# DuckTapeDevOps/kubernetes-cloud

Hardware: AMD Instinct MI355X
Metric: GPT-J-6B finetune tokens/sec (higher is better)
Workload: dtype bf16; 1 GPU; model=gpt-j-6b, global_batch=32, micro_batch=16, grad_accum=2, seq_len=2048, parallelism=dp1, activation_checkpointing=False

## Files before the change

csrc/kernels/attention_tiled.hip:

```cpp
#include "common.h"

#include <type_traits>

namespace {

constexpr float kLog2e = 1.4426950408889634f;
constexpr float kLn2 = 0.6931471805599453f;
constexpr float kRescaleThr = 8.0f;

#ifdef KCA_ATTN_STAMPS
__device__ unsigned long long g_attn_stamps[64];
__device__ __forceinline__ unsigned long long ast_now() {
  unsigned long long t;
  __builtin_amdgcn_sched_barrier(0);
  asm volatile("s_memtime %0\n\ts_waitcnt lgkmcnt(0)" : "=s"(t)::"memory");
  __builtin_amdgcn_sched_barrier(0);
  return t;
}
#define ASTAMP_DECL                                            \
  unsigned long long st_acc_[8] = {0, 0, 0, 0, 0, 0, 0, 0}; \
  unsigned long long st_prev_ = ast_now();
#define ASTAMP(k)                           \
  do {                                      \
    const unsigned long long n_ = ast_now(); \
    st_acc_[k] += n_ - st_prev_;            \
    st_prev_ = n_;                          \
  } while (0)
#define ASTAMP_FLUSH(base)                                                          \
  do {                                                                              \
    st_acc_[7] = 1;                                                                 \
    if ((threadIdx.x & 63) == 0)                                                    \
      for (int i_ = 0; i_ < 8; ++i_) atomicAdd(&g_attn_stamps[(base) + i_], st_acc_[i_]); \
  } while (0)
#else
#define ASTAMP_DECL
#define ASTAMP(k) \
  do {            \
  } while (0)
#define ASTAMP_FLUSH(base) \
  do {                     \
  } while (0)
#endif


struct FastFwdParams {
  const bf16_t* q; const bf16_t* k; const bf16_t* v;
  bf16_t* o; float* lse;
  int* flags;
  long long q_sb, q_st, q_sh, k_sb, k_st, k_sh, v_sb, v_st, v_sh;
  long long o_sb, o_st, o_sh;
  int B, Sq, Sk, H, Hkv;
  float scale;
};

typedef __attribute__((address_space(3))) bf16x4 lds_bf16x4_t;
typedef unsigned int u32x4 __attribute__((ext_vector_type(4)));

__device__ __forceinline__ bf16x4 lds_tr4(const char* base, int byte_off) {
  return __builtin_amdgcn_ds_read_tr16_b64_v4bf16(
      (lds_bf16x4_t*)(reinterpret_cast<uintptr_t>(base + byte_off)));
}

__device__ __forceinline__ bf16x8 lds_b128(const char* base, int byte_off) {
  return *reinterpret_cast<const bf16x8*>(base + byte_off);
}

template <int D>
__device__ __forceinline__ int img_off(int row, int ch) {
// ... 409 lines not shown
  u32x4 r;
#if defined(__HIP_DEVICE_COMPILE__)
  asm volatile("ds_read_b128 %0, %1 offset:%2" : "=v"(r) : "v"(addr), "i"(OFF));
#endif
  return r;
}
template <int OFF>
__device__ __forceinline__ u32x2 ads_tr(unsigned addr) {
  u32x2 r;
#if defined(__HIP_DEVICE_COMPILE__)
  asm volatile("ds_read_b64_tr_b16 %0, %1 offset:%2" : "=v"(r) : "v"(addr), "i"(OFF));
#endif
  return r;
}
template <int N>
__device__ __forceinline__ void lgkm_wait(u32x4& x) {
#if defined(__HIP_DEVICE_COMPILE__)
  asm volatile("s_waitcnt lgkmcnt(%1)" : "+v"(x) : "n"(N));
#endif
}
template <int N>
__device__ __forceinline__ void lgkm_wait(u32x2& x, u32x2& y, u32x2& z, u32x2& w) {
#if defined(__HIP_DEVICE_COMPILE__)
  asm volatile("s_waitcnt lgkmcnt(%4)" : "+v"(x), "+v"(y), "+v"(z), "+v"(w) : "n"(N));
#endif
}
__device__ __forceinline__ bf16x8 as_bf8(u32x4 x) { return *reinterpret_cast<bf16x8*>(&x); }
__device__ __forceinline__ bf16x8 as_bf8(u32x2 lo, u32x2 hi) {
  u32x4 x{lo[0], lo[1], hi[0], hi[1]};
  return *reinterpret_cast<bf16x8*>(&x);
}

template <int D, bool CAUSAL, int NW = 8, int NBUF = 4>
__global__ void __launch_bounds__(NW * 64, 1) attn_fwd_w8_kernel(FastFwdParams p) {
  constexpr int BM = NW * 32, BN = 32;
  constexpr int TILE = BN * D * 2;
  constexpr int STAGE = 2 * TILE;
  constexpr int KS = D / 16;
  constexpr int PIECES = TILE / 1024;
  constexpr int PPW = PIECES / NW;
  constexpr int LEAD = NBUF - 1;
  constexpr int INFLIGHT = (LEAD - 1) * 2 * PPW;
  static_assert(((D == 256 || D == 128) && NW == 8) || (D == 512 && NW == 4 && NBUF == 2 && !CAUSAL),
                "multi-wave LDS-DMA forward: 8 waves at D = 128 / 256, 4 waves at D = 512");
  static_assert(PPW >= 1 && PIECES % NW == 0, "whole pieces per wave");
  constexpr int SMEM = (NBUF * STAGE > NW * 32 * D * 2) ? NBUF * STAGE : NW * 32 * D * 2;
  __shared__ __attribute__((aligned(1024))) char smem[SMEM];

  const int tid = threadIdx.x, lane = tid & 63;
  const int wave = __builtin_amdgcn_readfirstlane(tid >> 6);
  const int l32 = lane & 31, hh = lane >> 5;
  const int nqb = p.Sq / BM;
  const int lid = xcd_remap(blockIdx.x, gridDim.x);
  const int qi = lid % nqb;
  const int qb = CAUSAL ? (nqb - 1 - qi) : qi;
  const int bh = lid / nqb;
  const int b = bh / p.H, h = bh % p.H;
  const int hk = h / (p.H / p.Hkv);
  const int off = p.Sk - p.Sq;
  const int q0 = qb * BM + wave * 32;
  const int qrow = q0 + l32;
  int kv_hi = p.Sk;
  if (CAUSAL) kv_hi = min(kv_hi, qb * BM + BM + off);
  const int ntiles = kv_hi / BN;
  const int mytiles = CAUSAL ? min(ntiles, (q0 + 32 + off) / BN) : ntiles;
  const float sl2 = p.scale * kLog2e;

  const bf16_t* qp = p.q + b * p.q_sb + h * p.q_sh;
  bf16x8 qf[KS];
#pragma unroll
  for (int s = 0; s < KS; ++s)
    qf[s] = *reinterpret_cast<const bf16x8*>(qp + (long long)qrow * p.q_st + 16 * s + 8 * hh);
  asm volatile("s_waitcnt vmcnt(0)" ::: "memory");

  const __amdgpu_buffer_rsrc_t rk = head_rsrc(p.k + b * p.k_sb + hk * p.k_sh);
  const __amdgpu_buffer_rsrc_t rv = head_rsrc(p.v + b * p.v_sb + hk * p.v_sh);
  static_assert((D / 64) % PPW == 0, "a wave's pieces within one row group");
  int kvo, vvo;
  {
    const int byte = 1024 * (wave * PPW) + 16 * lane;
    const int rg = byte / (16 * D), rem = byte % (16 * D);
    const int chh = rem / 512, w5 = rem % 512;
    const int row = rg * 8 + w5 / 64;
    const int ch = chh * 4 + (((w5 % 64) / 16) ^ ((row >> 2) & 3));
    kvo = (int)(((long long)row * p.k_st + ch * 8) * 2);
    vvo = (int)(((long long)row * p.v_st + ch * 8) * 2);
  }
  typedef __attribute__((address_space(3))) char lds_char;
  lds_char* lsm = (lds_char*)smem;
// ... 299 lines not shown
    {
      bf16x8 t0[2], t1[2];
      t0[0] = tr_frag<D>(Ks, b1, b2, 0, 0);
      t1[0] = tr_frag<D>(Ks, b1, b2, 1, 0);
      __builtin_amdgcn_sched_group_barrier(0x100, 4, 0);
#pragma unroll
      for (int db = 0; db < D / 32; ++db) {
        if (db + 1 < D / 32) {
          t0[(db + 1) & 1] = tr_frag<D>(Ks, b1, b2, 0, db + 1);
          t1[(db + 1) & 1] = tr_frag<D>(Ks, b1, b2, 1, db + 1);
          __builtin_amdgcn_sched_group_barrier(0x100, 4, 0);
        }
        dq[db] = __builtin_amdgcn_mfma_f32_32x32x16_bf16(t0[db & 1], d0, dq[db], 0, 0, 0);
        dq[db] = __builtin_amdgcn_mfma_f32_32x32x16_bf16(t1[db & 1], d1, dq[db], 0, 0, 0);
        __builtin_amdgcn_sched_group_barrier(0x8, 2, 0);
      }
    }
    ASTAMP(4);
    asm volatile("" ::: "memory");
    if (t + 1 < ntiles) stg.store(sk, sv, smem + ((t + 1) & 1) * 2 * TILE);
    __syncthreads();
    ASTAMP(5);
  };
  const int nfree = CAUSAL ? ntiles - 4 : ntiles;
  for (int t = 0; t < nfree; ++t) tile_step(t, std::false_type{});
  for (int t = max(nfree, 0); t < ntiles; ++t) tile_step(t, std::true_type{});
  store_tile_lds<D, DS>(p.dq + b * p.dq_sb + h * p.dq_sh + (long long)q0 * p.dq_st, p.dq_st, dq, lane, p.scale,
                        smem + wave * 32 * D * 2);
  ASTAMP(6);
  ASTAMP_FLUSH(16);
}

template <int D, bool CAUSAL>
__global__ void __launch_bounds__(256, 2) attn_bwd_dq_ds_kernel(FastBwdWsParams p) {
  constexpr int BM = 128, BN = 32;
  constexpr int TILE = BN * D * 2;
  constexpr int NCH = D / 8, CPT = 32 * NCH / 256, RPI = 256 / NCH;
  constexpr int DST = BN * 32 * 2;
  constexpr int DOFF = 2 * TILE;
  __shared__ __attribute__((aligned(16))) char smem[4 * TILE];
  static_assert(DOFF + 2 * 4 * DST <= 4 * TILE && 256 % NCH == 0, "dQ from dS: LDS plan");

  const int tid = threadIdx.x, lane = tid & 63, wave = tid >> 6;
  const int hh = lane >> 5;
  const int nqb = p.Sq / BM;
  const int lid = xcd_remap(blockIdx.x, gridDim.x);
  const int qi = lid % nqb;
  const int qb = CAUSAL ? (nqb - 1 - qi) : qi;
  const int bh = lid / nqb;
  const int b = bh / p.H, h = bh % p.H;
  const int off = p.Sk - p.Sq;
  const int q0 = qb * BM + wave * 32;
  int kv_hi = p.Sk;
  if (CAUSAL) kv_hi = min(kv_hi, qb * BM + BM + off);
  const int ntiles = (kv_hi + BN - 1) / BN;

  f32x16 dq[D / 32];
#pragma unroll
  for (int i = 0; i < D / 32; ++i)
#pragma unroll
    for (int r = 0; r < 16; ++r) dq[i][r] = 0.f;

  const __amdgpu_buffer_rsrc_t rk = head_rsrc(p.k + b * p.k_sb + h * p.k_sh);
  int vok[CPT], lk[CPT];
#pragma unroll
  for (int i = 0; i < CPT; ++i) {
    vok[i] = (int)(((long long)(tid / NCH + i * RPI) * p.k_st + (tid % NCH) * 8) * 2);
    lk[i] = img_off<D>(tid / NCH + i * RPI, tid % NCH);
  }
  const __amdgpu_buffer_rsrc_t rw = head_rsrc(p.ws + (long long)bh * p.Sq * p.Sk);
  const int ws_row = __builtin_amdgcn_readfirstlane((q0 / 32) * (p.Sk / 32) * DST);
  const int wv = lane * 16;
  char* const dsl = smem + DOFF + wave * DST;
  int dsw[4], dsr[4];
#pragma unroll
  for (int n = 0; n < 4; ++n) {
    const int l32 = lane & 31, key = 8 * n + 4 * hh + ((lane & 15) >> 2), qq = 4 * ((lane >> 4) & 1) + (lane & 3);
    dsw[n] = 64 * l32 + 8 * ((hh + 2 * n) ^ (l32 >> 2));
    dsr[n] = 64 * key + 8 * (qq ^ (key >> 2));
  }
  int b1, b2;
  tr_bases<D>(lane, b1, b2);

  constexpr int PD = 2;
  u32x4 sk[CPT], sd[PD][2];
  auto load_k = [&](int t) {
    const int sok = __builtin_amdgcn_readfirstlane((int)(t * BN * p.k_st * 2));
#pragma unroll
    for (int i = 0; i < CPT; ++i) {
      const auto a = __builtin_amdgcn_raw_buffer_load_b128(rk, vok[i], sok, 0);
      sk[i] = *reinterpret_cast<const u32x4*>(&a);
    }
  };
  auto load_ds = [&](int t, auto set) {
    const int so = __builtin_amdgcn_readfirstlane(ws_row + t * DST);
#pragma unroll
    for (int i = 0; i < 2; ++i) {
      const auto a = __builtin_amdgcn_raw_buffer_load_b128(rw, wv, so + i * (DST / 2), 2);
      sd[decltype(set)::value][i] = *reinterpret_cast<const u32x4*>(&a);
    }
  };
  auto store_tile = [&](int buf, auto set) {
    constexpr int J = decltype(set)::value;
#pragma unroll
    for (int i = 0; i < CPT; ++i) *reinterpret_cast<u32x4*>(smem + buf * TILE + lk[i]) = sk[i];
#pragma unroll
    for (int i = 0; i < 2; ++i) {
      *reinterpret_cast<u32x2*>(dsl + buf * 4 * DST + dsw[2 * i]) = u32x2{sd[J][i][0], sd[J][i][1]};
      *reinterpret_cast<u32x2*>(dsl + buf * 4 * DST + dsw[2 * i + 1]) = u32x2{sd[J][i][2], sd[J][i][3]};
    }
  };
  const int last = ntiles - 1;

  load_k(0);
  load_ds(0, std::integral_constant<int, 0>{});
  store_tile(0, std::integral_constant<int, 0>{});
  static_for<1, PD>([&](auto T) { load_ds(min(decltype(T)::value, last), T); });
  __builtin_amdgcn_sched_barrier(0);
  load_k(min(1, last));
  __builtin_amdgcn_sched_barrier(0);
  load_ds(min(PD, last), std::integral_constant<int, 0>{});
  __syncthreads();
  auto tile_step = [&](int t, auto jc) {
    constexpr int NX = (decltype(jc)::value + 1) % PD;
    const char* Ks = smem + (t & 1) * TILE;
    const char* ds = dsl + (t & 1) * 4 * DST;
    const bf16x8 d0 = cat8(lds_tr4(ds, dsr[0]), lds_tr4(ds, dsr[1]));
    const bf16x8 d1 = cat8(lds_tr4(ds, dsr[2]), lds_tr4(ds, dsr[3]));
    {
      bf16x8 t0[2], t1[2];
      t0[0] = tr_frag<D>(Ks, b1, b2, 0, 0);
      t1[0] = tr_frag<D>(Ks, b1, b2, 1, 0);
      __builtin_amdgcn_sched_group_barrier(0x100, 8, 0);
#pragma unroll
      for (int db = 0; db < D / 32; ++db) {
        if (db + 1 < D / 32) {
          t0[(db + 1) & 1] = tr_frag<D>(Ks, b1, b2, 0, db + 1);
          t1[(db + 1) & 1] = tr_frag<D>(Ks, b1, b2, 1, db + 1);
          __builtin_amdgcn_sched_group_barrier(0x100, 4, 0);
        }
        dq[db] = __builtin_amdgcn_mfma_f32_32x32x16_bf16(t0[db & 1], d0, dq[db], 0, 0, 0);
        dq[db] = __builtin_amdgcn_mfma_f32_32x32x16_bf16(t1[db & 1], d1, dq[db], 0, 0, 0);
        __builtin_amdgcn_sched_group_barrier(0x8, 2, 0);
      }
    }
    asm volatile("" ::: "memory");
    if (t + 1 < ntiles) store_tile((t + 1) & 1, std::integral_constant<int, NX>{});
    load_k(min(t + 2, last));
    load_ds(min(t + 1 + PD, last), std::integral_constant<int, NX>{});
    __syncthreads();
  };
  for (int t = 0; t < ntiles; t += PD)
    static_for<0, PD>([&](auto J) { tile_step(t + decltype(J)::value, J); });
  store_tile_lds<D>(p.dq + b * p.dq_sb + h * p.dq_sh + (long long)q0 * p.dq_st, p.dq_st, dq, lane, p.scale,
                    smem + wave * 32 * D * 2);
}

template <int D, bool CAUSAL, int DS = D>
__global__ void __launch_bounds__(256, (D <= 64 && !CAUSAL) ? 3 : 1) attn_bwd_dkdv_tiled_kernel(FastBwdParams p) {
  constexpr int BK = 128, BQ = 32;
  constexpr int TILE = BQ * D * 2;
  using Stg = StagerFor<D, DS>;
  constexpr int NCH = D / 8, NCS = DS / 8, CPT = Stg::CPT;
  constexpr int KSD = DS / 16;
  constexpr int VOFF = 4 * TILE;
  constexpr int LOFF = VOFF + 4 * TILE;
  __shared__ __attribute__((aligned(16))) char smem[LOFF + 2 * 64 * 4];
  ASTAMP_DECL

  const int tid = threadIdx.x, lane = tid & 63, wave = tid >> 6;
  const int l32 = lane & 31, hh = lane >> 5;
  const int nkb = p.Sk / BK;
  const int lid = xcd_remap(blockIdx.x, gridDim.x);
  const int kb = lid % nkb, bh = lid / nkb;
  const int b = bh / p.Hkv, hk = bh % p.Hkv;
  const int grp = p.H / p.Hkv;
  const int off = p.Sk - p.Sq;
  const int kw = kb * BK + wave * 32;
  const int key = kw + l32;
  const float sl2 = p.scale * kLog2e;

  const bf16_t* kp = p.k + b * p.k_sb + hk * p.k_sh;
  const bf16_t* vp = p.v + b * p.v_sb + hk * p.v_sh;
  bf16x8 kf[KSD];
#pragma unroll
  for (int s = 0; s < KSD; ++s)
    kf[s] = *reinterpret_cast<const bf16x8*>(kp + (long long)key * p.k_st + 16 * s + 8 * hh);
  char* vimg = smem + VOFF + wave * TILE;
// ... 153 lines not shown
    store_tile_lds<D, DS>(p.dk + b * p.dk_sb + hk * p.dk_sh + (long long)kw * p.dk_st, p.dk_st, dk, lane, p.scale,
                      smem + wave * 32 * D * 2);
    store_tile_lds<D, DS>(p.dv + b * p.dv_sb + hk * p.dv_sh + (long long)kw * p.dv_st, p.dv_st, dv, lane, 1.f,
                      smem + wave * 32 * D * 2);
  }
  ASTAMP(6);
  ASTAMP_FLUSH(32);
}

template <bool ON>
struct DsEmitter {
  __device__ __forceinline__ void init(const FastBwdParams&, int, int, int, int) {}
  __device__ __forceinline__ void store(const bf16x8&, const bf16x8&, int) const {}
};
template <>
struct DsEmitter<true> {
  __amdgpu_buffer_rsrc_t r_;
  int v_, dt_, t0_;
  __device__ __forceinline__ void init(const FastBwdWsParams& p, int bh, int lane, int q_lo, int kw) {
    r_ = head_rsrc(p.ws + (long long)bh * p.Sq * p.Sk);
    v_ = lane * 16;
    dt_ = (p.Sk / 32) * 2048;
    t0_ = (q_lo / 32) * dt_ + (kw / 32) * 2048;
  }
  __device__ __forceinline__ void store(const bf16x8& s0, const bf16x8& s1, int t) const {
    const int so = __builtin_amdgcn_readfirstlane(t0_ + t * dt_);
    __builtin_amdgcn_raw_buffer_store_b128(*reinterpret_cast<const u32x4*>(&s0), r_, v_, so, 2);
    __builtin_amdgcn_raw_buffer_store_b128(*reinterpret_cast<const u32x4*>(&s1), r_, v_, so + 1024, 2);
  }
};

template <int D, bool CAUSAL, bool EMIT_DS = false>
__global__ void __launch_bounds__(512, 1)
    attn_bwd_dkdv_w8_kernel(std::conditional_t<EMIT_DS, FastBwdWsParams, FastBwdParams> p) {
  constexpr int BK = 128, BQ = 32;
  constexpr int TILE = BQ * D * 2;
  using Stg = Stager<D, true, 512>;
  constexpr int CPT = Stg::CPT, KSD = D / 16;
  constexpr int PSZ = 4 * 64 * 16;
  constexpr int POFF = 3 * 2 * TILE;
  constexpr int LOFF = POFF + 2 * 4 * PSZ;
  __shared__ __attribute__((aligned(16))) char smem[LOFF + 3 * 64 * 4];
  static_assert(8 * 32 * D * 2 <= LOFF, "epilogue images of the 8 waves");
  ASTAMP_DECL

  const int tid = threadIdx.x, lane = tid & 63;
  const int wave = __builtin_amdgcn_readfirstlane(tid >> 6);
  const int pw = wave & 3;
  const bool kside = wave < 4;
  const int l32 = lane & 31, hh = lane >> 5;
  const int nkb = p.Sk / BK;
  const int lid = xcd_remap(blockIdx.x, gridDim.x);
  const int kb = lid % nkb, bh = lid / nkb;
  const int b = bh / p.H, h = bh % p.H;
  const int off = p.Sk - p.Sq;
  const int kw = kb * BK + pw * 32;
  const int key = kw + l32;
  const float sl2 = p.scale * kLog2e;

  bf16x8 rf[KSD];
  {
    const bf16_t* rp = kside ? p.v + b * p.v_sb + h * p.v_sh + (long long)key * p.v_st
                             : p.k + b * p.k_sb + h * p.k_sh + (long long)key * p.k_st;
#pragma unroll
    for (int s = 0; s < KSD; ++s) rf[s] = *reinterpret_cast<const bf16x8*>(rp + 16 * s + 8 * hh);
  }
  f32x16 acc[D / 32];
#pragma unroll
  for (int i = 0; i < D / 32; ++i)
#pragma unroll
    for (int r = 0; r < 16; ++r) acc[i][r] = 0.f;

  int q_lo = 0;
  if (CAUSAL) q_lo = max(0, kb * BK - off) & ~(BQ - 1);
  const int total = (p.Sq - q_lo) / BQ;

  const bf16_t* qb = p.q + b * p.q_sb + h * p.q_sh;
  const bf16_t* gb = p.dout + b * p.do_sb + h * p.do_sh;
  Stg stg(tid, p.q_st, p.do_st);
  stg.bind(qb, gb, p.q_st, p.do_st);
  u32x4 sq[CPT], sg[CPT];
  float lreg = 0.f;
  int be, bo, b1, b2;
  row_bases<D>(l32, hh, be, bo);
  tr_bases<D>(lane, b1, b2);

// ... 162 lines not shown
      __syncthreads();
      ASTAMP(5);
    };
    if (total > 1) {
      load_tile(1);
      store_tile(1);
    }
    __syncthreads();
    int cur = 0;
    for (int t = 0; t < total; ++t) {
      const int nxt = cur == 0 ? 2 : cur - 1;
      k_step(t, cur, nxt);
      cur = cur == 2 ? 0 : cur + 1;
    }
  }
  __builtin_amdgcn_s_setprio(0);
  {
    bf16_t* dst = kside ? p.dk + b * p.dk_sb + h * p.dk_sh + (long long)kw * p.dk_st
                        : p.dv + b * p.dv_sb + h * p.dv_sh + (long long)kw * p.dv_st;
    store_tile_lds<D>(dst, kside ? p.dk_st : p.dv_st, acc, lane, kside ? p.scale : 1.f, smem + wave * 32 * D * 2);
  }
  ASTAMP(6);
  if (!kside) {
    ASTAMP_FLUSH(40);
  } else {
    ASTAMP_FLUSH(56);
  }
}

inline bool offsets_fit(long long rows, long long stride) { return (rows + 128) * stride * 2 < (1ll << 31); }

}

static int g_attn_variant = 7;
KCA_API int kca_attn_set_variant(int v) {
  g_attn_variant = v;
  return 0;
}

KCA_API int kca_attn_fwd_tiled(const void* q, const void* k, const void* v, void* o, float* lse,
                               long long q_sb, long long q_st, long long q_sh, long long k_sb,
                               long long k_st, long long k_sh, long long v_sb, long long v_st,
                               long long v_sh, long long o_sb, long long o_st, long long o_sh,
                               int B, int Sq, int Sk, int H, int Hkv, int d, int causal,
                               float scale, int rowsum_col, int max_col, int* flags, hipStream_t stream) {
  if ((d != 48 && d != 64 && d != 96 && d != 128 && d != 160 && d != 256) || Sq % 128 || Sk % 32 || Sq <= 0 ||
      H % Hkv || !flags)
    return 1;
  if (max_col >= 0 && (max_col != 40 || rowsum_col != 40 || d != 48)) return 1;
  if (d == 48 && causal) return 1;
  if (rowsum_col >= 0 && (rowsum_col != 40 || (d != 64 && d != 48) || causal)) return 1;
  if (causal && Sk < Sq) return 1;
  if (!offsets_fit(Sk, k_st) || !offsets_fit(Sk, v_st)) return 1;
  FastFwdParams p{(const bf16_t*)q, (const bf16_t*)k, (const bf16_t*)v, (bf16_t*)o, lse, flags,
                  q_sb, q_st, q_sh, k_sb, k_st, k_sh, v_sb, v_st, v_sh, o_sb, o_st, o_sh,
                  B, Sq, Sk, H, Hkv, scale};
  dim3 grid((Sq / 128) * B * H);
  (void)hipGetLastError();
  if (d == 256 && (g_attn_variant & 1) && Sq % 256 == 0) {
    dim3 g8((Sq / 256) * B * H);
    if (causal) hipLaunchKernelGGL((attn_fwd_w8_kernel<256, true>), g8, dim3(512), 0, stream, p);
    else hipLaunchKernelGGL((attn_fwd_w8_kernel<256, false>), g8, dim3(512), 0, stream, p);
  } else if (d == 256) {
    if (causal) hipLaunchKernelGGL((attn_fwd_tiled_kernel<256, true>), grid, dim3(256), 0, stream, p);
    else hipLaunchKernelGGL((attn_fwd_tiled_kernel<256, false>), grid, dim3(256), 0, stream, p);
  } else if (d == 160) {
    if (causal) hipLaunchKernelGGL((attn_fwd_tiled_kernel<160, true>), grid, dim3(256), 0, stream, p);
    else hipLaunchKernelGGL((attn_fwd_tiled_kernel<160, false>), grid, dim3(256), 0, stream, p);
  } else if (d == 128) {
    if (causal) hipLaunchKernelGGL((attn_fwd_tiled_kernel<128, true>), grid, dim3(256), 0, stream, p);
    else hipLaunchKernelGGL((attn_fwd_tiled_kernel<128, false>), grid, dim3(256), 0, stream, p);
  } else if (d == 96) {
    if (causal) hipLaunchKernelGGL((attn_fwd_tiled_kernel<96, true>), grid, dim3(256), 0, stream, p);
    else hipLaunchKernelGGL((attn_fwd_tiled_kernel<96, false>), grid, dim3(256), 0, stream, p);
  } else if (d == 48) {
    if (max_col == 40) hipLaunchKernelGGL((attn_fwd_tiled_kernel<64, false, 40, 48, 40>), grid, dim3(256), 0, stream, p);
    else if (rowsum_col == 40) hipLaunchKernelGGL((attn_fwd_tiled_kernel<64, false, 40, 48>), grid, dim3(256), 0, stream, p);
    else hipLaunchKernelGGL((attn_fwd_tiled_kernel<64, false, -1, 48>), grid, dim3(256), 0, stream, p);
  } else {
    if (causal) hipLaunchKernelGGL((attn_fwd_tiled_kernel<64, true>), grid, dim3(256), 0, stream, p);
    else if (rowsum_col == 40) hipLaunchKernelGGL((attn_fwd_tiled_kernel<64, false, 40>), grid, dim3(256), 0, stream, p);
    else hipLaunchKernelGGL((attn_fwd_tiled_kernel<64, false>), grid, dim3(256), 0, stream, p);
  }
  return hipGetLastError() == hipSuccess ? 0 : 3;
}

KCA_API int kca_attn_fwd_wide(const void* q, const void* k, const void* v, void* o, float* lse, long long q_sb,
                              long long q_st, long long q_sh, long long k_sb, long long k_st, long long k_sh,
                              long long v_sb, long long v_st, long long v_sh, long long o_sb, long long o_st,
                              long long o_sh, int B, int Sq, int Sk, int H, int Hkv, int d, float scale, int* flags,
                              hipStream_t stream) {
  if (d != 512 || Sq % 128 || Sk % 32 || Sq <= 0 || Sk <= 0 || H % Hkv || !flags) return 1;
  if (!offsets_fit(Sk, k_st) || !offsets_fit(Sk, v_st)) return 1;
  if ((q_st | k_st | v_st | o_st) % 8) return 1;
  FastFwdParams p{(const bf16_t*)q, (const bf16_t*)k, (const bf16_t*)v, (bf16_t*)o, lse, flags,
                  q_sb, q_st, q_sh, k_sb, k_st, k_sh, v_sb, v_st, v_sh, o_sb, o_st, o_sh,
                  B, Sq, Sk, H, Hkv, scale};
  (void)hipGetLastError();
  hipLaunchKernelGGL((attn_fwd_w8_kernel<512, false, 4, 2>), dim3((Sq / 128) * B * H), dim3(256), 0, stream, p);
  return hipGetLastError() == hipSuccess ? 0 : 3;
}

KCA_API int kca_attn_bwd_tiled(const void* q, const void* k, const void* v, const void* dout,
                               void* dq, void* dk, void* dv, const float* lse, const float* delta,
                               long long q_sb, long long q_st, long long q_sh, long long k_sb,
                               long long k_st, long long k_sh, long long v_sb, long long v_st,
                               long long v_sh, long long do_sb, long long do_st, long long do_sh,
                               long long dq_sb, long long dq_st, long long dq_sh, long long dk_sb,
                               long long dk_st, long long dk_sh, long long dv_sb, long long dv_st,
                               long long dv_sh, int B, int Sq, int Sk, int H, int Hkv, int d,
                               int causal, float scale, hipStream_t stream) {
  if ((d != 48 && d != 64 && d != 96 && d != 128 && d != 160 && d != 256) || Sq % 128 || Sk % 128 || Sq <= 0 ||
      H % Hkv)
    return 1;
  if (d == 48 && causal) return 1;
  if (causal && Sk < Sq) return 1;
  if (!offsets_fit(Sk, k_st) || !offsets_fit(Sk, v_st) || !offsets_fit(Sq, q_st) || !offsets_fit(Sq, do_st)) return 1;
  FastBwdParams p{(const bf16_t*)q, (const bf16_t*)k, (const bf16_t*)v, (const bf16_t*)dout,
                  (bf16_t*)dq, (bf16_t*)dk, (bf16_t*)dv, lse, delta,
                  q_sb, q_st, q_sh, k_sb, k_st, k_sh, v_sb, v_st, v_sh, do_sb, do_st, do_sh,
                  dq_sb, dq_st, dq_sh, dk_sb, dk_st, dk_sh, dv_sb, dv_st, dv_sh,
                  B, Sq, Sk, H, Hkv, scale};
  dim3 g1((Sk / 128) * B * Hkv), g2((Sq / 128) * B * H);
  if (d == 48) {
    hipLaunchKernelGGL((attn_bwd_dkdv_tiled_kernel<64, false, 48>), g1, dim3(256), 0, stream, p);
    hipLaunchKernelGGL((attn_bwd_dq_tiled_kernel<64, false, 48>), g2, dim3(256), 0, stream, p);
  } else if (d == 256) {
    const bool w8 = (g_attn_variant & 2) && H == Hkv;
    if (causal) {
      if (w8) hipLaunchKernelGGL((attn_bwd_dkdv_w8_kernel<256, true>), g1, dim3(512), 0, stream, p);
      else hipLaunchKernelGGL((attn_bwd_dkdv_tiled_kernel<256, true>), g1, dim3(256), 0, stream, p);
      hipLaunchKernelGGL((attn_bwd_dq_tiled_kernel<256, true>), g2, dim3(256), 0, stream, p);
    } else {
      if (w8) hipLaunchKernelGGL((attn_bwd_dkdv_w8_kernel<256, false>), g1, dim3(512), 0, stream, p);
      else hipLaunchKernelGGL((attn_bwd_dkdv_tiled_kernel<256, false>), g1, dim3(256), 0, stream, p);
      hipLaunchKernelGGL((attn_bwd_dq_tiled_kernel<256, false>), g2, dim3(256), 0, stream, p);
    }
  } else if (d == 160) {
    if (causal) {
      hipLaunchKernelGGL((attn_bwd_dkdv_tiled_kernel<160, true>), g1, dim3(256), 0, stream, p);
      hipLaunchKernelGGL((attn_bwd_dq_tiled_kernel<160, true>), g2, dim3(256), 0, stream, p);
    } else {
      hipLaunchKernelGGL((attn_bwd_dkdv_tiled_kernel<160, false>), g1, dim3(256), 0, stream, p);
      hipLaunchKernelGGL((attn_bwd_dq_tiled_kernel<160, false>), g2, dim3(256), 0, stream, p);
    }
  } else if (d == 96) {
    if (causal) {
      hipLaunchKernelGGL((attn_bwd_dkdv_tiled_kernel<96, true>), g1, dim3(256), 0, stream, p);
      hipLaunchKernelGGL((attn_bwd_dq_tiled_kernel<96, true>), g2, dim3(256), 0, stream, p);
    } else {
      hipLaunchKernelGGL((attn_bwd_dkdv_tiled_kernel<96, false>), g1, dim3(256), 0, stream, p);
      hipLaunchKernelGGL((attn_bwd_dq_tiled_kernel<96, false>), g2, dim3(256), 0, stream, p);
    }
  } else if (d == 128) {
    if (causal) {
      hipLaunchKernelGGL((attn_bwd_dkdv_tiled_kernel<128, true>), g1, dim3(256), 0, stream, p);
      hipLaunchKernelGGL((attn_bwd_dq_tiled_kernel<128, true>), g2, dim3(256), 0, stream, p);
    } else {
      hipLaunchKernelGGL((attn_bwd_dkdv_tiled_kernel<128, false>), g1, dim3(256), 0, stream, p);
      hipLaunchKernelGGL((attn_bwd_dq_tiled_kernel<128, false>), g2, dim3(256), 0, stream, p);
    }
  } else {
    if (causal) {
      hipLaunchKernelGGL((attn_bwd_dkdv_tiled_kernel<64, true>), g1, dim3(256), 0, stream, p);
      hipLaunchKernelGGL((attn_bwd_dq_tiled_kernel<64, true>), g2, dim3(256), 0, stream, p);
    } else {
      hipLaunchKernelGGL((attn_bwd_dkdv_tiled_kernel<64, false>), g1, dim3(256), 0, stream, p);
// ... 2 lines not shown
  }
  return 0;
}

KCA_API long long kca_attn_bwd_ws_bytes(int B, int Sq, int Sk, int H, int Hkv, int d, int causal) {
  if (d != 256 || H != Hkv || B <= 0 || H <= 0 || Sq <= 0 || Sq % 128 || Sk % 128 || (causal && Sk < Sq)) return 0;
  if ((long long)Sq * Sk * 2 >= (1ll << 31)) return 0;
  return (long long)B * H * Sq * Sk * 2;
}

KCA_API int kca_attn_bwd_tiled_ws(const void* q, const void* k, const void* v, const void* dout,
                                  void* dq, void* dk, void* dv, const float* lse, const float* delta,
                                  long long q_sb, long long q_st, long long q_sh, long long k_sb,
                                  long long k_st, long long k_sh, long long v_sb, long long v_st,
                                  long long v_sh, long long do_sb, long long do_st, long long do_sh,
                                  long long dq_sb, long long dq_st, long long dq_sh, long long dk_sb,
                                  long long dk_st, long long dk_sh, long long dv_sb, long long dv_st,
                                  long long dv_sh, int B, int Sq, int Sk, int H, int Hkv, int d,
                                  int causal, float scale, void* ws, long long ws_bytes, hipStream_t stream) {
  const long long need = kca_attn_bwd_ws_bytes(B, Sq, Sk, H, Hkv, d, causal);
  if ((g_attn_variant & 6) != 6 || !ws || need == 0 || ws_bytes < need || !offsets_fit(Sk, k_st) ||
      !offsets_fit(Sk, v_st) || !offsets_fit(Sq, q_st) || !offsets_fit(Sq, do_st))
    return kca_attn_bwd_tiled(q, k, v, dout, dq, dk, dv, lse, delta, q_sb, q_st, q_sh, k_sb, k_st, k_sh, v_sb,
                              v_st, v_sh, do_sb, do_st, do_sh, dq_sb, dq_st, dq_sh, dk_sb, dk_st, dk_sh, dv_sb,
                              dv_st, dv_sh, B, Sq, Sk, H, Hkv, d, causal, scale, stream);
  FastBwdWsParams p{{(const bf16_t*)q, (const bf16_t*)k, (const bf16_t*)v, (const bf16_t*)dout,
                     (bf16_t*)dq, (bf16_t*)dk, (bf16_t*)dv, lse, delta,
                     q_sb, q_st, q_sh, k_sb, k_st, k_sh, v_sb, v_st, v_sh, do_sb, do_st, do_sh,
                     dq_sb, dq_st, dq_sh, dk_sb, dk_st, dk_sh, dv_sb, dv_st, dv_sh,
                     B, Sq, Sk, H, Hkv, scale},
                    (bf16_t*)ws};
  dim3 g1((Sk / 128) * B * H), g2((Sq / 128) * B * H);
  if (causal) {
    hipLaunchKernelGGL((attn_bwd_dkdv_w8_kernel<256, true, true>), g1, dim3(512), 0, stream, p);
    hipLaunchKernelGGL((attn_bwd_dq_ds_kernel<256, true>), g2, dim3(256), 0, stream, p);
  } else {
    hipLaunchKernelGGL((attn_bwd_dkdv_w8_kernel<256, false, true>), g1, dim3(512), 0, stream, p);
    hipLaunchKernelGGL((attn_bwd_dq_ds_kernel<256, false>), g2, dim3(256), 0, stream, p);
  }
  return 0;
}

#ifdef KCA_ATTN_STAMPS
KCA_API int kca_attn_stamps(unsigned long long* host, int reset) {
  if (hipMemcpyFromSymbol(host, HIP_SYMBOL(g_attn_stamps), sizeof(unsigned long long) * 64) != hipSuccess) return 1;
  if (reset) {
    unsigned long long z[64] = {0};
    if (hipMemcpyToSymbol(HIP_SYMBOL(g_attn_stamps), z, sizeof(z)) != hipSuccess) return 1;
  }
  return 0;
}
#endif
```

kubernetes_cloud_amd/ops/_lib.py:

```python
from __future__ import annotations

import ctypes
import os
import threading

import torch

_HERE = os.path.dirname(os.path.abspath(__file__))
LIB_DIR = os.path.join(os.path.dirname(_HERE), "_lib")
DEBUG = os.environ.get("KCA_DEBUG", "0") in ("1", "true")
KERNEL_LIB = os.path.join(LIB_DIR, "libkca_kernels_debug.so" if DEBUG else "libkca_kernels.so")
KERNEL_LIB = os.environ.get("KCA_KERNEL_LIB") or KERNEL_LIB
ATTN_VARIANT_ENV = os.environ.get("KCA_ATTN_VARIANT")

_lock = threading.Lock()
_lib = None
_err: str | None = None

P = ctypes.c_void_p
I = ctypes.c_int
LL = ctypes.c_longlong
F = ctypes.c_float

_SIGS = {
    "kca_layernorm_fwd": [P, P, P, P, P, P, P, P, P, I, I, F, P],
    "kca_gemm_lt": [P, LL, P, LL, P, P, LL, P, LL, I, I, I, F, P, LL, P],
    "kca_gemm_lt_gelu": [P, LL, P, LL, I, P, P, LL, P, LL, I, I, I, P, LL, P],
    "kca_layernorm_bwd_parts": [I],
    "kca_layernorm_bwd": [P, P, P, P, P, P, P, P, P, I, P, I, I, P],
    "kca_gelu_fwd": [P, P, LL, I, P],
    "kca_gelu_fwd_f16": [P, P, LL, I, P],
    "kca_gelu_bwd": [P, P, P, LL, I, P],
    "kca_quick_gelu_fwd": [P, P, LL, P],
    "kca_quick_gelu_bwd": [P, P, P, LL, P],
    "kca_geglu_fwd": [P, P, LL, I, P],
    "kca_add_bias_nhwc": [P, P, P, P, LL, I, P],
    "kca_add_bias2_nhwc": [P, P, P, P, P, LL, I, P],
    "kca_colsum_bf16": [P, P, I, I, I, P],
    "kca_geglu_bwd": [P, P, P, LL, I, P],
    "kca_rope": [P, P, I, I, LL, I, LL, LL, LL, LL, I, I, P, P, P, F, P],
    "kca_accum_grad": [P, P, F, I, LL, P],
    "kca_accum_grad_pair": [P, P, P, F, LL, P],
    "kca_accum_grad_multi": [P, I, F, P],
    "kca_cast_f32_bf16": [P, P, LL, P],
    "kca_ema": [P, P, F, LL, P],
    "kca_cross_entropy_fwd": [P, LL, P, I, I, I, P, P, P],
    "kca_cross_entropy_bwd": [P, LL, P, P, P, F, I, I, I, P, LL, P],
    "kca_adamw": [P, P, P, P, P, LL, P, F, F, F, F, F, F, F, P, P, P],
    "kca_sumsq": [P, LL, P, P, P],
    "kca_adamw8bit": [P, P, P, P, P, P, P, LL, P, F, F, F, F, F, F, F, P, P, P],
    "kca_clip_coef": [P, F, F, P, P, P, P],
    "kca_attn_fwd": [P] * 5 + [LL] * 12 + [I] * 7 + [F, P, P, I, P, I, I, P, P],
    "kca_attn_bwd_preprocess": [P, P, P, LL, LL, LL, LL, LL, LL, I, I, I, I, P],
    "kca_attn_bwd": [P] * 10 + [LL] * 21 + [I] * 7 + [F, P, P, I, P, P],
    "kca_attn_bwd_ws": [P] * 10 + [LL] * 21 + [I] * 7 + [F, P, P, I, P, P, LL, P],
    "kca_attn_bwd_ws_bytes": [I] * 7,
    "kca_attn_fwd_wide": [P] * 5 + [LL] * 12 + [I] * 6 + [F, P, P],
    "kca_attn_set_tiled": [I],
    "kca_attn_set_variant": [I],
    "kca_transpose_bf16": [P, LL, P, LL, I, I, P],
    "kca_gelu_fwd_t": [P, LL, P, LL, P, LL, I, I, I, P],
    "kca_gelu_bwd_t": [P, LL, P, LL, P, LL, P, LL, P, I, I, I, P],
    "kca_transpose_colsum": [P, LL, P, LL, P, I, I, P],
    "kca_col_reduce_f32": [P, I, I, P, P, P],
    "kca_accum_grad_2d": [P, P, LL, I, I, F, I, P],
    "kca_groupnorm_fwd": [P, P, P, P, P, P, P, I, I, I, I, F, I, P],
    "kca_groupnorm_bwd": [P, P, P, P, P, P, P, P, P, P, I, I, I, I, I, P],
    "kca_groupnorm_nhwc_ws": [I, I, I],
    "kca_groupnorm_nhwc_fwd": [P, P, P, P, P, P, P, I, I, I, I, F, I, P],
    "kca_groupnorm_nhwc_fwd_add": [P, P, P, P, LL, P, P, P, P, I, I, I, I, F, I, P],
    "kca_groupnorm_nhwc_cat_fwd": [P, P, P, P, P, P, P, P, P, P, I, I, I, I, I, I, F, I, P],
    "kca_groupnorm_nhwc_bwd": [P, P, P, P, P, P, P, P, P, P, I, I, I, I, I, P],
    "kca_skinny_set_smallk": [I],
    "kca_conv3x3_fwd": [P, P, P, P, I, I, I, I, I, P],
    "kca_conv3x3_set_variant": [I],
    "kca_conv3x3_wflip": [P, P, I, I, P],
    "kca_conv3x3_wgrad_splits": [I, I, I, I, I],
    "kca_conv3x3_wgrad": [P, P, P, P, I, I, I, I, I, I, P],
    "kca_skinny_gemm": [P, LL, P, P, P, LL, I, I, I, I, P],
    "kca_skinny_set_splitk": [I],
    "kca_w8_gemm": [P, LL, P, P, P, P, LL, I, I, I, I, I, P],
    "kca_w8_set_kgroups": [I],
    "kca_mx4_gemm": [P, LL, P, P, P, P, LL, I, I, I, I, I, P],
    "kca_kv8_prep": [P, LL, I, I, I, I, I, I, P, P, P, P, P, P, P, P, LL, LL, LL, LL, LL, P, I, I, I, P],
    "kca_kv8_attn": [P, LL, P, P, P, P, LL, LL, LL, LL, LL, P, P, P, LL, P, LL, I, I, I, I, I, I, F, P, P, I, I, I,
                     I, P],
    "kca_mm_skinny_set": [I],
    "kca_ln_skinny_gemm": [P, LL, P, P, P, LL, P, P, F, P, P, P, LL, I, I, I, I, P, P],
    "kca_ln_rows": [P, LL, P, P, P, LL, P, P, F, P, I, I, P],
    "kca_embed_ln_rows": [P, LL, P, P, P, I, P, LL, P, P, F, P, I, I, P],
    "kca_decode_prep": [P, LL, I, I, I, I, I, I, P, P, P, P, P, P, LL, LL, LL, P, I, I, P],
    "kca_decode_chunk": [I, I, I],
# ... 18 lines not shown

_RESTYPES = {"kca_attn_bwd_ws_bytes": ctypes.c_longlong}

_SIGS["kca_decode_prep_attn_gemv"] = _SIGS["kca_decode_prep_attn"][:-2] + [P, P, P, P, I, I, I, I, P]

for _n in ("kca_decode_prep_attn", "kca_ln_rows", "kca_embed_ln_rows", "kca_decode_prep_attn_gemv",
           "kca_gemv_dual_ln", "kca_skinny_gemm"):
    _SIGS[_n + "_f16"] = _SIGS[_n]


def _load():
    global _lib, _err
    if _lib is not None or _err is not None:
        return _lib
    with _lock:
        if _lib is not None or _err is not None:
            return _lib
        if not os.path.exists(KERNEL_LIB):
            _err = f"{KERNEL_LIB} not built (run `python tools/build_ext.py`)"
            return None
        try:
            lib = ctypes.CDLL(KERNEL_LIB, mode=ctypes.RTLD_GLOBAL)
        except OSError as e:
            _err = f"failed to load {KERNEL_LIB}: {e}"
            return None
        for name, argtypes in _SIGS.items():
            fn = getattr(lib, name, None)
            if fn is None:
                continue
            fn.argtypes = argtypes
            fn.restype = _RESTYPES.get(name, ctypes.c_int)
        if ATTN_VARIANT_ENV is not None and hasattr(lib, "kca_attn_set_variant"):
            lib.kca_attn_set_variant(int(ATTN_VARIANT_ENV))
        _lib = lib
        return _lib


def available() -> bool:
    return _load() is not None


def require():
    lib = _load()
    if lib is None:
        raise RuntimeError(
            "kubernetes_cloud_amd native kernels unavailable: " + str(_err)
            + " -- refusing to fall back to eager PyTorch on a GPU tensor")
    return lib


def has(name: str) -> bool:
    lib = _load()
    return lib is not None and hasattr(lib, name)


SYNC_LAUNCH = os.environ.get("KCA_SYNC_LAUNCH", "0") in ("1", "true")


LAUNCHES = [0]


def call(name: str, *args):
    lib = require()
    fn = getattr(lib, name)
    LAUNCHES[0] += 1
    rc = fn(*args)
# ... 45 lines not shown
```

kubernetes_cloud_amd/ops/attention.py:

```python
from __future__ import annotations

import math

import torch

from . import _lib
from .rope import apply_rotary_


def attention_reference(q, k, v, causal: bool, scale: float | None = None,
                        kv_len: torch.Tensor | None = None, alibi: torch.Tensor | None = None,
                        window: int = 0):
    B, Sq, H, D = q.shape
    Sk, Hkv = k.shape[1], k.shape[2]
    scale = scale if scale is not None else 1.0 / math.sqrt(D)
    qf = q.float().transpose(1, 2)
    kf = k.float().transpose(1, 2)
    vf = v.float().transpose(1, 2)
    if Hkv != H:
        rep = H // Hkv
        kf = kf.repeat_interleave(rep, dim=1)
        vf = vf.repeat_interleave(rep, dim=1)
    s = torch.matmul(qf, kf.transpose(-1, -2)) * scale
    qi = torch.arange(Sq, device=q.device)[:, None]
    ki = torch.arange(Sk, device=q.device)[None, :]
    off = Sk - Sq
    if alibi is not None:
        s = s + alibi.float().view(1, H, 1, 1) * (ki - qi - off).float()
    mask = torch.zeros(B, 1, Sq, Sk, dtype=torch.bool, device=q.device)
    if causal:
        mask = mask | (ki > qi + off)
    if window:
        mask = mask | (ki <= qi + off - window)
    if kv_len is not None and kv_len.dtype == torch.bool:
        mask = mask | ~kv_len.to(q.device).view(B, 1, 1, Sk)
    elif kv_len is not None:
        mask = mask | (ki[None, None] >= kv_len.view(B, 1, 1, 1).to(q.device))
    s = s.masked_fill(mask, float("-inf"))
    lse = torch.logsumexp(s, dim=-1)
    p = torch.exp(s - lse[..., None])
    p = torch.nan_to_num(p, nan=0.0)
    o = torch.matmul(p, vf).transpose(1, 2)
    return o.to(q.dtype), lse


def set_tiled_path(enable: bool) -> None:
    _lib.call("kca_attn_set_tiled", int(bool(enable)))


DEFAULT_VARIANT = 7
_VARIANT = [int(_lib.ATTN_VARIANT_ENV) if _lib.ATTN_VARIANT_ENV is not None else DEFAULT_VARIANT]


def set_variant(v: int) -> int:
    _lib.call("kca_attn_set_variant", int(v))
    old, _VARIANT[0] = _VARIANT[0], int(v)
    return old


def _strides(t):
    return t.stride(0), t.stride(1), t.stride(2)


def pack_key_mask(mask: torch.Tensor) -> torch.Tensor:
    B, Sk = mask.shape
    W = (Sk + 31) // 32
    m = torch.zeros(B, W * 32, dtype=torch.int64, device=mask.device)
    m[:, :Sk] = mask.to(torch.int64)
    words = (m.view(B, W, 32) << torch.arange(32, device=mask.device, dtype=torch.int64)).sum(-1)
    words = torch.where(words >= 2 ** 31, words - 2 ** 32, words)
    return words.to(torch.int32).contiguous()


def _masks(kv_len):
    if kv_len is None:
        return None, None
    return (kv_len, None) if kv_len.dim() == 1 else (None, kv_len)


def _fwd(q, k, v, causal, scale, kv_len, alibi, out=None, window: int = 0, rowsum_col: int = -1,
         max_col: int = -1, lse=None, flags=None):
    B, Sq, H, D = q.shape
    Sk, Hkv = k.shape[1], k.shape[2]
    o = out if out is not None else torch.empty(B, Sq, H, D, device=q.device, dtype=q.dtype)
    if lse is None:
        lse = torch.empty(B, H, Sq, device=q.device, dtype=torch.float32)
    if flags is None:
        flags = torch.empty(4 * ((Sq + 127) // 128) * B * H, device=q.device, dtype=torch.int32)
    lens, km = _masks(kv_len)
    _lib.call("kca_attn_fwd", q.data_ptr(), k.data_ptr(), v.data_ptr(), o.data_ptr(), lse.data_ptr(),
# ... 169 lines not shown
```

Before: 36130 tokens/s.

## Interleave tail heads in causal attention block order to balance XCD load

Replaces the plain XCD remap in the causal D=256 forward, dK/dV and dQ-from-dS kernels with a block order that, within each XCD's contiguous chunk, interleaves the last few heads by block row. The aim is to stop the final heavy causal blocks of several heads landing at the end of the schedule, which leaves CUs idle at the tail of each launch. The default variant gains bit 8 to turn this on, with configurable tail-head counts per kernel. Timing stamp hooks are also added to the dQ kernel but compile away by default.

```diff
diff --git a/csrc/kernels/attention_tiled.hip b/csrc/kernels/attention_tiled.hip
--- a/csrc/kernels/attention_tiled.hip
+++ b/csrc/kernels/attention_tiled.hip
@@ -1,4 +1,5 @@
 #include "common.h"
+#include "block_order.h"
 
 #include <type_traits>
 
@@ -32,8 +33,12 @@
     if ((threadIdx.x & 63) == 0)                                                    \
       for (int i_ = 0; i_ < 8; ++i_) atomicAdd(&g_attn_stamps[(base) + i_], st_acc_[i_]); \
   } while (0)
+#define ASTAMP_VMWAIT(n) asm volatile("s_waitcnt vmcnt(%0)" ::"n"(n) : "memory")
 #else
 #define ASTAMP_DECL
+#define ASTAMP_VMWAIT(n) \
+  do {                   \
+  } while (0)
 #define ASTAMP(k) \
   do {            \
   } while (0)
@@ -509,7 +514,8 @@
 }
 
 template <int D, bool CAUSAL, int NW = 8, int NBUF = 4>
-__global__ void __launch_bounds__(NW * 64, 1) attn_fwd_w8_kernel(FastFwdParams p) {
+__global__ void __launch_bounds__(NW * 64, 1)
+    attn_fwd_w8_kernel(FastFwdParams p, int tail_heads) {
   constexpr int BM = NW * 32, BN = 32;
   constexpr int TILE = BN * D * 2;
   constexpr int STAGE = 2 * TILE;
@@ -528,10 +534,10 @@
   const int wave = __builtin_amdgcn_readfirstlane(tid >> 6);
   const int l32 = lane & 31, hh = lane >> 5;
   const int nqb = p.Sq / BM;
-  const int lid = xcd_remap(blockIdx.x, gridDim.x);
-  const int qi = lid % nqb;
+  const BlockOrder ord = causal_block_order(blockIdx.x, gridDim.x, nqb, (CAUSAL && D == 256) ? tail_heads : 0);
+  const int qi = ord.blk;
   const int qb = CAUSAL ? (nqb - 1 - qi) : qi;
-  const int bh = lid / nqb;
+  const int bh = ord.bh;
   const int b = bh / p.H, h = bh % p.H;
   const int hk = h / (p.H / p.Hkv);
   const int off = p.Sk - p.Sq;
@@ -897,7 +903,7 @@
 }
 
 template <int D, bool CAUSAL>
-__global__ void __launch_bounds__(256, 2) attn_bwd_dq_ds_kernel(FastBwdWsParams p) {
+__global__ void __launch_bounds__(256, 2) attn_bwd_dq_ds_kernel(FastBwdWsParams p, int tail_heads) {
   constexpr int BM = 128, BN = 32;
   constexpr int TILE = BN * D * 2;
   constexpr int NCH = D / 8, CPT = 32 * NCH / 256, RPI = 256 / NCH;
@@ -909,10 +915,10 @@
   const int tid = threadIdx.x, lane = tid & 63, wave = tid >> 6;
   const int hh = lane >> 5;
   const int nqb = p.Sq / BM;
-  const int lid = xcd_remap(blockIdx.x, gridDim.x);
-  const int qi = lid % nqb;
+  const BlockOrder ord = causal_block_order(blockIdx.x, gridDim.x, nqb, (CAUSAL && D == 256) ? tail_heads : 0);
+  const int qi = ord.blk;
   const int qb = CAUSAL ? (nqb - 1 - qi) : qi;
-  const int bh = lid / nqb;
+  const int bh = ord.bh;
   const int b = bh / p.H, h = bh % p.H;
   const int off = p.Sk - p.Sq;
   const int q0 = qb * BM + wave * 32;
@@ -976,6 +982,7 @@
     }
   };
   const int last = ntiles - 1;
+  ASTAMP_DECL
 
   load_k(0);
   load_ds(0, std::integral_constant<int, 0>{});
@@ -986,6 +993,7 @@
   __builtin_amdgcn_sched_barrier(0);
   load_ds(min(PD, last), std::integral_constant<int, 0>{});
   __syncthreads();
+  ASTAMP(0);
   auto tile_step = [&](int t, auto jc) {
     constexpr int NX = (decltype(jc)::value + 1) % PD;
     const char* Ks = smem + (t & 1) * TILE;
@@ -1010,15 +1018,25 @@
       }
     }
     asm volatile("" ::: "memory");
+    ASTAMP(1);
+    ASTAMP_VMWAIT(2 * (PD - 1) + CPT);
+    ASTAMP(2);
+    ASTAMP_VMWAIT(2 * (PD - 1));
+    ASTAMP(3);
     if (t + 1 < ntiles) store_tile((t + 1) & 1, std::integral_constant<int, NX>{});
+    ASTAMP(4);
     load_k(min(t + 2, last));
     load_ds(min(t + 1 + PD, last), std::integral_constant<int, NX>{});
+    ASTAMP(5);
     __syncthreads();
+    ASTAMP(6);
   };
   for (int t = 0; t < ntiles; t += PD)
     static_for<0, PD>([&](auto J) { tile_step(t + decltype(J)::value, J); });
   store_tile_lds<D>(p.dq + b * p.dq_sb + h * p.dq_sh + (long long)q0 * p.dq_st, p.dq_st, dq, lane, p.scale,
                     smem + wave * 32 * D * 2);
+  ASTAMP(0);
+  ASTAMP_FLUSH(24);
 }
 
 template <int D, bool CAUSAL, int DS = D>
@@ -1238,7 +1256,7 @@
 
 template <int D, bool CAUSAL, bool EMIT_DS = false>
 __global__ void __launch_bounds__(512, 1)
-    attn_bwd_dkdv_w8_kernel(std::conditional_t<EMIT_DS, FastBwdWsParams, FastBwdParams> p) {
+    attn_bwd_dkdv_w8_kernel(std::conditional_t<EMIT_DS, FastBwdWsParams, FastBwdParams> p, int tail_heads) {
   constexpr int BK = 128, BQ = 32;
   constexpr int TILE = BQ * D * 2;
   using Stg = Stager<D, true, 512>;
@@ -1256,8 +1274,8 @@
   const bool kside = wave < 4;
   const int l32 = lane & 31, hh = lane >> 5;
   const int nkb = p.Sk / BK;
-  const int lid = xcd_remap(blockIdx.x, gridDim.x);
-  const int kb = lid % nkb, bh = lid / nkb;
+  const BlockOrder ord = causal_block_order(blockIdx.x, gridDim.x, nkb, (CAUSAL && D == 256) ? tail_heads : 0);
+  const int kb = ord.blk, bh = ord.bh;
   const int b = bh / p.H, h = bh % p.H;
   const int off = p.Sk - p.Sq;
   const int kw = kb * BK + pw * 32;
@@ -1486,11 +1504,29 @@
 
 }
 
-static int g_attn_variant = 7;
+static int g_attn_variant = 15;
 KCA_API int kca_attn_set_variant(int v) {
   g_attn_variant = v;
   return 0;
 }
+
+static int g_attn_tail[3] = {32, 8, 4};
+KCA_API int kca_attn_set_block_order(int fwd_tail, int dkdv_tail, int dq_tail) {
+  if (fwd_tail >= 0) g_attn_tail[0] = fwd_tail;
+  if (dkdv_tail >= 0) g_attn_tail[1] = dkdv_tail;
+  if (dq_tail >= 0) g_attn_tail[2] = dq_tail;
+  return 0;
+}
+static inline int attn_tail(int kernel) { return (g_attn_variant & 8) ? g_attn_tail[kernel] : 0; }
+
+KCA_API int kca_attn_block_order(int bid, int grid, int nblk, int tail_heads, int* bh, int* blk) {
+  if (!bh || !blk || nblk <= 0 || grid <= 0 || grid % nblk || bid < 0 || bid >= grid) return 1;
+  const BlockOrder ord = causal_block_order(bid, grid, nblk, tail_heads);
+  *bh = ord.bh;
+  *blk = ord.blk;
+  return 0;
+}
+KCA_API int kca_attn_get_tail_heads(int kernel) { return (kernel < 0 || kernel > 2) ? -1 : g_attn_tail[kernel]; }
 
 KCA_API int kca_attn_fwd_tiled(const void* q, const void* k, const void* v, void* o, float* lse,
                                long long q_sb, long long q_st, long long q_sh, long long k_sb,
@@ -1513,8 +1549,8 @@
   (void)hipGetLastError();
   if (d == 256 && (g_attn_variant & 1) && Sq % 256 == 0) {
     dim3 g8((Sq / 256) * B * H);
-    if (causal) hipLaunchKernelGGL((attn_fwd_w8_kernel<256, true>), g8, dim3(512), 0, stream, p);
-    else hipLaunchKernelGGL((attn_fwd_w8_kernel<256, false>), g8, dim3(512), 0, stream, p);
+    if (causal) hipLaunchKernelGGL((attn_fwd_w8_kernel<256, true>), g8, dim3(512), 0, stream, p, attn_tail(0));
+    else hipLaunchKernelGGL((attn_fwd_w8_kernel<256, false>), g8, dim3(512), 0, stream, p, 0);
   } else if (d == 256) {
     if (causal) hipLaunchKernelGGL((attn_fwd_tiled_kernel<256, true>), grid, dim3(256), 0, stream, p);
     else hipLaunchKernelGGL((attn_fwd_tiled_kernel<256, false>), grid, dim3(256), 0, stream, p);
@@ -1551,7 +1587,7 @@
                   q_sb, q_st, q_sh, k_sb, k_st, k_sh, v_sb, v_st, v_sh, o_sb, o_st, o_sh,
                   B, Sq, Sk, H, Hkv, scale};
   (void)hipGetLastError();
-  hipLaunchKernelGGL((attn_fwd_w8_kernel<512, false, 4, 2>), dim3((Sq / 128) * B * H), dim3(256), 0, stream, p);
+  hipLaunchKernelGGL((attn_fwd_w8_kernel<512, false, 4, 2>), dim3((Sq / 128) * B * H), dim3(256), 0, stream, p, 0);
   return hipGetLastError() == hipSuccess ? 0 : 3;
 }
 
@@ -1582,11 +1618,11 @@
   } else if (d == 256) {
     const bool w8 = (g_attn_variant & 2) && H == Hkv;
     if (causal) {
-      if (w8) hipLaunchKernelGGL((attn_bwd_dkdv_w8_kernel<256, true>), g1, dim3(512), 0, stream, p);
+      if (w8) hipLaunchKernelGGL((attn_bwd_dkdv_w8_kernel<256, true>), g1, dim3(512), 0, stream, p, attn_tail(1));
       else hipLaunchKernelGGL((attn_bwd_dkdv_tiled_kernel<256, true>), g1, dim3(256), 0, stream, p);
       hipLaunchKernelGGL((attn_bwd_dq_tiled_kernel<256, true>), g2, dim3(256), 0, stream, p);
     } else {
-      if (w8) hipLaunchKernelGGL((attn_bwd_dkdv_w8_kernel<256, false>), g1, dim3(512), 0, stream, p);
+      if (w8) hipLaunchKernelGGL((attn_bwd_dkdv_w8_kernel<256, false>), g1, dim3(512), 0, stream, p, 0);
       else hipLaunchKernelGGL((attn_bwd_dkdv_tiled_kernel<256, false>), g1, dim3(256), 0, stream, p);
       hipLaunchKernelGGL((attn_bwd_dq_tiled_kernel<256, false>), g2, dim3(256), 0, stream, p);
     }
@@ -1655,11 +1691,11 @@
                     (bf16_t*)ws};
   dim3 g1((Sk / 128) * B * H), g2((Sq / 128) * B * H);
   if (causal) {
-    hipLaunchKernelGGL((attn_bwd_dkdv_w8_kernel<256, true, true>), g1, dim3(512), 0, stream, p);
-    hipLaunchKernelGGL((attn_bwd_dq_ds_kernel<256, true>), g2, dim3(256), 0, stream, p);
+    hipLaunchKernelGGL((attn_bwd_dkdv_w8_kernel<256, true, true>), g1, dim3(512), 0, stream, p, attn_tail(1));
+    hipLaunchKernelGGL((attn_bwd_dq_ds_kernel<256, true>), g2, dim3(256), 0, stream, p, attn_tail(2));
   } else {
-    hipLaunchKernelGGL((attn_bwd_dkdv_w8_kernel<256, false, true>), g1, dim3(512), 0, stream, p);
-    hipLaunchKernelGGL((attn_bwd_dq_ds_kernel<256, false>), g2, dim3(256), 0, stream, p);
+    hipLaunchKernelGGL((attn_bwd_dkdv_w8_kernel<256, false, true>), g1, dim3(512), 0, stream, p, 0);
+    hipLaunchKernelGGL((attn_bwd_dq_ds_kernel<256, false>), g2, dim3(256), 0, stream, p, 0);
   }
   return 0;
 }
diff --git a/csrc/kernels/block_order.h b/csrc/kernels/block_order.h
--- /dev/null
+++ b/csrc/kernels/block_order.h
@@ -0,0 +1,40 @@
+#pragma once
+
+#if defined(__HIPCC__)
+#define KCA_BO_HD __host__ __device__ __forceinline__
+#else
+#define KCA_BO_HD inline
+#endif
+
+struct BlockOrder {
+  int bh;
+  int blk;
+};
+
+KCA_BO_HD BlockOrder causal_block_order(int bid, int grid, int nblk, int tail_heads) {
+  const int full = grid & ~7;
+  if (bid >= full) return {bid / nblk, bid % nblk};
+  const int cs = full >> 3, lo = (bid & 7) * cs;
+  const int lid = lo + (bid >> 3);
+  const BlockOrder same{lid / nblk, lid % nblk};
+  if (tail_heads <= 0) return same;
+  const int end = lo + cs - 1;
+  const int h0 = lo / nblk, h1 = end / nblk;
+  const int e = end - h1 * nblk;
+  const int hs = (h1 - h0 < tail_heads) ? h0 : h1 - tail_heads + 1;
+  int ts = hs * nblk, a = 0;
+  if (ts < lo) {
+    a = lo - ts;
+    ts = lo;
+  }
+  if (lid < ts) return same;
+  int k = lid - ts;
+  const int nh = h1 - hs + 1;
+  for (int r = 0; r < nblk; ++r) {
+    const int skip = r < a ? 1 : 0;
+    const int c = nh - skip - (r > e ? 1 : 0);
+    if (k < c) return {hs + skip + k, r};
+    k -= c;
+  }
+  return same;
+}
diff --git a/kubernetes_cloud_amd/ops/_lib.py b/kubernetes_cloud_amd/ops/_lib.py
--- a/kubernetes_cloud_amd/ops/_lib.py
+++ b/kubernetes_cloud_amd/ops/_lib.py
@@ -12,6 +12,7 @@
 KERNEL_LIB = os.path.join(LIB_DIR, "libkca_kernels_debug.so" if DEBUG else "libkca_kernels.so")
 KERNEL_LIB = os.environ.get("KCA_KERNEL_LIB") or KERNEL_LIB
 ATTN_VARIANT_ENV = os.environ.get("KCA_ATTN_VARIANT")
+ATTN_TAIL_ENV = os.environ.get("KCA_ATTN_TAIL_HEADS")
 
 _lock = threading.Lock()
 _lib = None
@@ -58,6 +59,9 @@
     "kca_attn_fwd_wide": [P] * 5 + [LL] * 12 + [I] * 6 + [F, P, P],
     "kca_attn_set_tiled": [I],
     "kca_attn_set_variant": [I],
+    "kca_attn_set_block_order": [I, I, I],
+    "kca_attn_get_tail_heads": [I],
+    "kca_attn_block_order": [I, I, I, I, P, P],
     "kca_transpose_bf16": [P, LL, P, LL, I, I, P],
     "kca_gelu_fwd_t": [P, LL, P, LL, P, LL, I, I, I, P],
     "kca_gelu_bwd_t": [P, LL, P, LL, P, LL, P, LL, P, I, I, I, P],
@@ -142,6 +146,9 @@
             fn.restype = _RESTYPES.get(name, ctypes.c_int)
         if ATTN_VARIANT_ENV is not None and hasattr(lib, "kca_attn_set_variant"):
             lib.kca_attn_set_variant(int(ATTN_VARIANT_ENV))
+        if ATTN_TAIL_ENV is not None and hasattr(lib, "kca_attn_set_block_order"):
+            t = [int(x) for x in ATTN_TAIL_ENV.split(",")]
+            lib.kca_attn_set_block_order(*(t * 3 if len(t) == 1 else t))
         _lib = lib
         return _lib
 
diff --git a/kubernetes_cloud_amd/ops/attention.py b/kubernetes_cloud_amd/ops/attention.py
--- a/kubernetes_cloud_amd/ops/attention.py
+++ b/kubernetes_cloud_amd/ops/attention.py
@@ -48,7 +48,7 @@
     _lib.call("kca_attn_set_tiled", int(bool(enable)))
 
 
-DEFAULT_VARIANT = 7
+DEFAULT_VARIANT = 15
 _VARIANT = [int(_lib.ATTN_VARIANT_ENV) if _lib.ATTN_VARIANT_ENV is not None else DEFAULT_VARIANT]
 
 
@@ -56,6 +56,25 @@
     _lib.call("kca_attn_set_variant", int(v))
     old, _VARIANT[0] = _VARIANT[0], int(v)
     return old
+
+
+def set_block_order(fwd_tail: int = -1, dkdv_tail: int = -1, dq_tail: int = -1) -> None:
+    _lib.call("kca_attn_set_block_order", int(fwd_tail), int(dkdv_tail), int(dq_tail))
+
+
+def tail_heads() -> tuple[int, int, int]:
+    lib = _lib.require()
+    return tuple(lib.kca_attn_get_tail_heads(i) for i in range(3))
+
+
+def block_order(bid: int, grid: int, nblk: int, tail: int) -> tuple[int, int]:
+    import ctypes
+
+    bh, blk = ctypes.c_int(), ctypes.c_int()
+    rc = _lib.require().kca_attn_block_order(bid, grid, nblk, tail, ctypes.byref(bh), ctypes.byref(blk))
+    if rc != 0:
+        raise ValueError(f"kca_attn_block_order({bid}, {grid}, {nblk}, {tail}) returned {rc}")
+    return bh.value, blk.value
 
 
 def _strides(t):
```

Result: no change. 36450 tokens/s, median of 6 (+0.9%).
